# Arshardh/siddhi

Measured on AMD Instinct MI355X. Metric: events/sec (node) windowed group-by agg at 1/2/4/8 GPUs; % HBM roofline, higher is better.
Workload: dtype f64; 1 GPU; C2 timeBatch(1 sec) count/min/max/avg group by k, per-event sends; key_type=string (dictionary ids = dense slots), keys_per_gpu=100000, keys_total=100000, send_size=1, parallelism=key-sharded x1, flushes=69793, rows=6978983088

## Files before the change

siddhi_amd/csrc/sh_internal.h:

```cpp
#pragma once

#include <hip/hip_runtime.h>
#include <stdint.h>

#include "../../include/siddhi_hip.h"

namespace shd {

typedef unsigned long long u64;
typedef int64_t i64;
typedef unsigned int u32;

constexpr int kMaxFilterOps = 32;
constexpr int kBlock = 256;
constexpr int kItems = 8;
constexpr int kTile = kBlock * kItems;
constexpr u64 kEmptyKey = 0x8000000000000001ull;
constexpr u32 kNoPos = 0xFFFFFFFFu;
constexpr int kPackIdxBits = 22;
constexpr u32 kPackIdxMask = (1u << kPackIdxBits) - 1u;

struct FilterOpD {
    int op, type, col, pad;
    i64 ival;
// ... 156 lines not shown
                        WinParams wp, PushInfo* info, i64* blk_xm = nullptr, ColSet cols = ColSet{});
void launch_boundaries(hipStream_t s, const i64* ts, ColSet cols, FilterProg f, WinParams wp,
                       i64* blk_pass_pre, const i64* blk_tl_pre, PushInfo* info, Bound* bounds,
                       int max_bounds, int nblk, KeyPlan kp, KeyTable kt, u32* new_pos, const i64* blk_xm_pre = nullptr,
                       u32* ms_counts = nullptr, int P = 1, int ms_nblk = 0, int ms_col0 = 0, bool sorted = false,
                       i64* scan_tmp = nullptr);
int agg_unit_rows(int P, int NL, bool own);
void launch_aggregate(hipStream_t s, const Segment* segs, int nseg, int P, int logP, int NL, i64 n_pend,
                      const u32* pend_pos, const u64* pend_vals, i64 pend_cap, const u32* new_pos, ColSet cols,
                      AggPlan ap, u64* rows, int RW, u32* unit_rows, u32* first_bits,
                      const u32* rec_pos, const u32* rec_idx, const u64* rec_vals, i64 rec_cap, const i64* seg_off,
                      bool pack, EvSrc es, bool dense_rows = false,
                      bool persistent = true);
void launch_count_flags(hipStream_t s, const unsigned char* flags, i64 n, i64* blk_cnt, int nblk);
void launch_scan_sum(hipStream_t s, i64* a, int n);
void launch_bits_prefix(hipStream_t s, const u32* bits, i64 nw, i64* tile_sum, u64* word_pre, u32* total);
void launch_emit_rows(hipStream_t s, const u64* rows, int RW, const u32* unit_rows, i64 n_units, int unit_stride,
                      i64 row_cap, const u32* n_rows_dev, const u64* word_pre, int n_aggs, KeyTable kt,
                      KeyPlan kp, i64 n_pend, const i64* pend_ts, const i64* ts, i64 out_cap, i64* out_ts,
                      i64* out_keys, u64* out_vals, const u64* pend_gidx, const u64* new_gidx, i64* out_order,
                      i64 seq_base, i64* out_rep, u64* stage);
size_t emit_stage_bytes(int nk, int na, int order, i64 n_rows);
void launch_emit_gather(hipStream_t s, const u64* word_pre, i64 nw, const Segment* segs, int nseg, int P, int logP,
                        int unit_stride, const u64* rows, int RW, PosSrc ps, const u32* pend_pos, i64 n_pend,
                        const u32* n_rows_dev, int n_aggs, KeyTable kt, KeyPlan kp, i64* out_ts, i64* out_keys,
                        u64* out_vals, const u64* pend_gidx, const u64* new_gidx, i64* out_order, i64 seq_base,
                        i64* out_rep);
void launch_compact_pending(hipStream_t s, const i64* ts, ColSet cols, PosSrc new_pos, AggPlan ap, i64 e_lo,
                            i64 N, i64 pcb_lo, i64 base, const i64* blk_pass_pre, u32* pend_pos, i64* pend_ts,
                            u64* pend_vals, i64 pend_cap, const u64* new_gidx, u64* pend_gidx, i64 seq_base);
constexpr int kSmallT = 1024;
// ... 214 lines not shown
```

siddhi_amd/csrc/sh_kernels.hip:

```cpp
#include "sh_device.h"

namespace shd {

#ifdef SH_STAMPS
constexpr int kStampKernels = 4, kStampBlocks = 32768, kStampPts = 16;
__device__ unsigned long long g_stamps[kStampKernels * kStampBlocks * kStampPts];
#define SH_STAMP_AT(kern, idx, pt, WAIT)                                                                     \
    do {                                                                                                     \
        if (threadIdx.x == 0 && (idx) < kStampBlocks) {                                                      \
            asm volatile(WAIT ::: "memory");                                                                 \
            g_stamps[((size_t)(kern) * kStampBlocks + (idx)) * kStampPts + (pt)] = __builtin_amdgcn_s_memtime(); \
        }                                                                                                    \
    } while (0)
#define SH_STAMP(kern, pt) SH_STAMP_AT(kern, blockIdx.x, pt, "s_waitcnt vmcnt(0) lgkmcnt(0)")
#define SH_STAMP_UNIT(kern, unit, pt) SH_STAMP_AT(kern, unit, pt, "s_waitcnt vmcnt(0) lgkmcnt(0)")
#define SH_STAMP_UNIT_LDS(kern, unit, pt) SH_STAMP_AT(kern, unit, pt, "s_waitcnt lgkmcnt(0)")
#else
#define SH_STAMP(kern, pt) do {} while (0)
#define SH_STAMP_UNIT(kern, unit, pt) do {} while (0)
#define SH_STAMP_UNIT_LDS(kern, unit, pt) do {} while (0)
#endif

template <int FK>
__global__ __launch_bounds__(kBlock) void k_blockagg(const i64* __restrict__ ts, ColSet cols, FilterProg f,
// ... 899 lines not shown

void launch_scan_sum(hipStream_t s, i64* a, int n) {
    hipLaunchKernelGGL(k_scan_sum, dim3(1), dim3(1024), 0, s, a, n);
}

__global__ __launch_bounds__(kBlock) void k_bits_tile(const u32* __restrict__ bits, i64 nw, i64* tile_sum) {
    const i64 base = (i64)blockIdx.x * kTile + (i64)threadIdx.x * kItems;
    i64 c = 0;
#pragma unroll
    for (int i = 0; i < kItems; i++) if (base + i < nw) c += __popc(bits[base + i]);
    const i64 t = block_reduce(c, SumOp(), 0);
    if (threadIdx.x == 0) tile_sum[blockIdx.x] = t;
}

__global__ __launch_bounds__(kBlock) void k_bits_pre(const u32* __restrict__ bits, i64 nw, const i64* tile_pre,
                                                    u64* word_pre, u32* total) {
    const i64 base = (i64)blockIdx.x * kTile + (i64)threadIdx.x * kItems;
    u32 b[kItems];
    i64 c = 0;
#pragma unroll
    for (int i = 0; i < kItems; i++) { b[i] = base + i < nw ? bits[base + i] : 0; c += __popc(b[i]); }
    i64 r = block_excl_scan(c, SumOp(), 0, nullptr) + tile_pre[blockIdx.x];
#pragma unroll
    for (int i = 0; i < kItems; i++) {
        if (base + i < nw) word_pre[base + i] = ((u64)b[i] << 32) | (u32)r;
        r += __popc(b[i]);
        if (base + i == nw - 1) *total = (u32)r;
    }
}

void launch_bits_prefix(hipStream_t s, const u32* bits, i64 nw, i64* tile_sum, u64* word_pre, u32* total) {
    const int nb = (int)((nw + kTile - 1) / kTile);
    hipLaunchKernelGGL(k_bits_tile, dim3(nb), dim3(kBlock), 0, s, bits, nw, tile_sum);
    launch_scan_sum(s, tile_sum, nb);
    hipLaunchKernelGGL(k_bits_pre, dim3(nb), dim3(kBlock), 0, s, bits, nw, tile_sum, word_pre, total);
}

__host__ __device__ constexpr int stage_words(int nk, int na, int order) { return (2 + nk + order + na + 1) & ~1; }

constexpr int kStageMax = 2 + kKeyParts + 1 + SH_MAX_AGGS + 1;
__global__ __launch_bounds__(kBlock) void k_emit_rank(const u64* __restrict__ rows, int RW,
                                                     const u32* __restrict__ unit_rows, i64 n_units,
                                                     int unit_stride,
                                                     const u64* __restrict__ word_pre,
                                                     int n_aggs, KeyTable kt, KeyPlan kp, i64 n_pend,
                                                     const i64* __restrict__ pend_ts, const i64* __restrict__ ts,
                                                     const u64* __restrict__ pend_gidx,
                                                     const u64* __restrict__ new_gidx, int want_order, i64 seq_base,
                                                     u64* stage) {
    __shared__ ulonglong2 sw[kBlock][kStageMax / 2];
// ... 506 lines not shown
    if (p <= P) part_off[p] = counts[(i64)p * nblk];
}

void launch_part_off(hipStream_t s, const i64* counts, int nblk, int P, i64* part_off) {
    hipLaunchKernelGGL(k_part_off, dim3((P + 1 + 255) / 256), dim3(256), 0, s, counts, nblk, P, part_off);
}

constexpr int kColT = 16;
__global__ __launch_bounds__(kBlock) void k_col_reduce(const u32* __restrict__ c, int nblk, int P, i64* bsum,
                                                      u32* ticket) {
    const int b = blockIdx.y;
    const int p = blockIdx.x * kBlock + threadIdx.x;
    if (b == 0 && p == 0) *ticket = 0;
    if (p >= P) return;
    const int t0 = b * kColT, t1 = min(nblk, t0 + kColT);
    i64 acc = 0;
    for (int t = t0; t < t1; t++) acc += c[(i64)t * P + p];
    bsum[(i64)b * P + p] = acc;
}

__global__ __launch_bounds__(kBlock) void k_col_blocks(i64* bsum, int nb, int P, i64* total, i64* base, u32* ticket) {
    const int p = blockIdx.x;
    i64 run = 0;
    for (int b0 = 0; b0 < nb; b0 += kBlock) {
        const int b = b0 + threadIdx.x;
        const i64 x = b < nb ? bsum[(i64)b * P + p] : 0;
        i64 tot;
        const i64 pre = block_excl_scan(x, SumOp(), 0, &tot);
        if (b < nb) bsum[(i64)b * P + p] = run + pre;
        run += tot;
    }
    __shared__ bool last;
    if (threadIdx.x == 0) {
        total[p] = run;
        __threadfence();
        last = atomicAdd(ticket, 1u) == (u32)(P - 1);
    }
    __syncthreads();
    if (!last) return;
    __threadfence();
    i64 carry = 0;
    for (int q0 = 0; q0 < P; q0 += kBlock) {
        const int q = q0 + threadIdx.x;
        const i64 x = q < P ? __atomic_load_n(&total[q], __ATOMIC_RELAXED) : 0;
        i64 tot;
        const i64 pre = block_excl_scan(x, SumOp(), 0, &tot);
        if (q < P) base[q] = carry + pre;
        carry += tot;
    }
}

__global__ __launch_bounds__(kBlock) void k_col_walk(i64* __restrict__ bsum, int nb, int P, i64* __restrict__ total,
                                                    i64* __restrict__ base) {
    const int p = blockIdx.x * kBlock + threadIdx.x;
    if (p >= P) return;
    i64 run = 0;
    for (int b0 = 0; b0 < nb; b0 += 8) {
        i64 x[8];
#pragma unroll
        for (int k = 0; k < 8; k++) x[k] = b0 + k < nb ? bsum[(i64)(b0 + k) * P + p] : 0;
#pragma unroll
        for (int k = 0; k < 8; k++) {
            if (b0 + k < nb) bsum[(i64)(b0 + k) * P + p] = run;
            run += x[k];
        }
    }
    total[p] = run;
    base[p] = run;
}

__global__ __launch_bounds__(kBlock) void k_col_apply(u32* c, int nblk, int P, const i64* __restrict__ bpre,
                                                     const i64* __restrict__ base, const i64* __restrict__ total) {
    const int b = blockIdx.y;
    const int p = blockIdx.x * kBlock + threadIdx.x;
    if (p >= P) return;
    const int t0 = b * kColT, t1 = min(nblk, t0 + kColT);
    i64 run = base[p] + bpre[(i64)b * P + p];
    for (int t = t0; t < t1; t++) {
        const u32 x = c[(i64)t * P + p];
        c[(i64)t * P + p] = (u32)run;
        run += x;
    }
    if (t1 == nblk) c[(i64)nblk * P + p] = (u32)(base[p] + total[p]);
}

size_t ms_offsets_tmp_bytes(int nblk, int P) {
    const size_t nb = (size_t)(std::max(nblk, 1) + kColT - 1) / kColT;
    return (nb * P + 2 * (size_t)P + 16) * 8;
}

void launch_ms_offsets(hipStream_t s, u32* counts, int nblk, int P, i64* tmp) {
    const int nb = (std::max(nblk, 1) + kColT - 1) / kColT;
    i64* bsum = tmp;
    i64* total = tmp + (size_t)nb * P;
    i64* base = total + P;
    u32* ticket = (u32*)(base + P);
    const dim3 g((P + kBlock - 1) / kBlock, nb);
    hipLaunchKernelGGL(k_col_reduce, g, dim3(kBlock), 0, s, counts, nblk, P, bsum, ticket);
    if (P >= 2048 && nb <= 256) {
        hipLaunchKernelGGL(k_col_walk, dim3((P + kBlock - 1) / kBlock), dim3(kBlock), 0, s, bsum, nb, P, total, base);
        launch_scan_sum(s, base, P);
    } else {
        hipLaunchKernelGGL(k_col_blocks, dim3(P), dim3(kBlock), 0, s, bsum, nb, P, total, base, ticket);
    }
    if (nblk > 0) hipLaunchKernelGGL(k_col_apply, g, dim3(kBlock), 0, s, counts, nblk, P, bsum, base, total);
    else hipLaunchKernelGGL(k_col_apply, dim3((P + kBlock - 1) / kBlock, 1), dim3(kBlock), 0, s, counts, nblk, P, bsum,
                            base, total);
}

__global__ __launch_bounds__(kBlock) void k_seg_offsets(const Segment* __restrict__ segs, int nseg, i64 n_pend,
                                                       const u32* __restrict__ pend_pos,
                                                       PosSrc new_pos, int P,
                                                       const u32* __restrict__ counts, TileMap m, i64* seg_off) {
    extern __shared__ __attribute__((aligned(16))) u32 hist[];
    const int k = blockIdx.x;
    const i64 b = k < nseg ? segs[k].lo : segs[nseg - 1].hi;
    const int t = tile_of(m, b);
    for (int i = threadIdx.x; i < P; i += kBlock) hist[i] = 0;
// ... 636 lines not shown
```

siddhi_amd/csrc/sh_runtime.cpp:

```cpp
#include <hip/hip_runtime.h>

#include <algorithm>
#include <cstdio>
#include <cstdlib>
#include <cstring>
#include <string>
#include <vector>

#include "sh_agg.h"
#include "sh_internal.h"
#include "sh_runtime.h"

#include <chrono>

using namespace shd;

thread_local std::string g_last_error;

int sh_fail(int code, const std::string& msg) {
    g_last_error = msg;
    SH_TRACE("error %d: %s", code, msg.c_str());
    return code;
}

// ... 93 lines not shown
}

void DevBuf::release() {
    if (p) {
        (void)drain();
        (void)hipFree(p);
    }
    p = nullptr;
    cap = used = 0;
}

int PinnedBuf::reserve(size_t n) {
    if (n <= cap) return SH_OK;
    release();
    size_t ncap = std::max<size_t>(n, 4096);
    if (hipHostMalloc(&p, ncap, hipHostMallocDefault) != hipSuccess) {
        p = nullptr;
        return sh_fail(SH_ERR_OOM, "pinned host allocation failed");
    }
    cap = ncap;
    return SH_OK;
}

void PinnedBuf::release() {
    if (p) (void)hipHostFree(p);
    p = nullptr;
    cap = 0;
}

extern "C" int sh_init(int32_t device, sh_ctx** out) {
    if (!out) return sh_fail(SH_ERR_INVALID, "sh_init: out is NULL");
    int n = 0;
    hipError_t e = hipGetDeviceCount(&n);
    if (e != hipSuccess || n == 0) return sh_fail(SH_ERR_DEVICE, "no HIP device visible (this library has no CPU path)");
    if (device < 0 || device >= n) return sh_fail(SH_ERR_INVALID, "sh_init: bad device ordinal");
    HIPCHK(hipSetDevice(device));
    hipDeviceProp_t prop;
    HIPCHK(hipGetDeviceProperties(&prop, device));
    if (std::string(prop.gcnArchName).find("gfx950") == std::string::npos)
        return sh_fail(SH_ERR_DEVICE, std::string("built for gfx950, found ") + prop.gcnArchName);
    hipMemPool_t pool = nullptr;
// ... 287 lines not shown
```

siddhi_amd/csrc/sh_runtime.h:

```cpp
#pragma once

#include <hip/hip_runtime.h>
#include <rocprofiler-sdk-roctx/roctx.h>

#include <algorithm>
#include <cstdio>
#include <new>
#include <utility>
#include <string>
#include <unordered_map>
#include <vector>

#include "sh_internal.h"
#include "sh_having.h"

struct sh_ctx {
    int device = 0;
    int num_cus = 0;
    int max_lds = 0;
    hipStream_t stream = nullptr;
    hipStream_t copy_stream = nullptr;
    hipStream_t side_stream = nullptr;
};

// ... 49 lines not shown
            release();
            p = o.p; cap = o.cap; used = o.used;
            o.p = nullptr; o.cap = o.used = 0;
        }
        return *this;
    }
    ~DevBuf() { release(); }
    int reserve(size_t n, bool keep);
    void release();
    template <typename T> T* as() const { return (T*)p; }
};

struct PinnedBuf {
    void* p = nullptr;
    size_t cap = 0;
    PinnedBuf() = default;
    PinnedBuf(const PinnedBuf&) = delete;
    PinnedBuf& operator=(const PinnedBuf&) = delete;
    PinnedBuf(PinnedBuf&& o) noexcept : p(o.p), cap(o.cap) { o.p = nullptr; o.cap = 0; }
    PinnedBuf& operator=(PinnedBuf&& o) noexcept {
        if (this != &o) {
            release();
            p = o.p; cap = o.cap;
            o.p = nullptr; o.cap = 0;
        }
        return *this;
    }
    ~PinnedBuf() { release(); }
    int reserve(size_t n);
    void release();
    template <typename T> T* as() const { return (T*)p; }
};

struct KeyTableHost {
    DevBuf keys, ctrl;
    PinnedBuf h_ctrl;
    size_t size_ = 0;
    int64_t n_keys = 0;
    bool reserved_used = false;
// ... 158 lines not shown
    DevBuf pend_pos, pend_ts, pend_vals;
    DevBuf pend_tmp;
    DevBuf sp_pos, sp_ts, sp_vals, sp_gidx;
    int64_t sp_cap = 0;
    bool side_push = false;
    DevBuf blk_pass, blk_tl, blk_first, blk_xm, info, bounds, segs, seg_rows, rows, counters, out_ts, out_keys, out_vals,
        out_nulls, out_expired, out_rep, blk_cnt;
    DevBuf first_bits, word_pre;
    DevBuf emit_stage;
    const void* zeroed_nulls = nullptr;
    const void* zeroed_expired = nullptr;
    DevBuf ms_counts, ms_tmp, rec_pos, rec_idx, rec_vals, part_off;
    DevBuf new_pos, seg_off;
    PushInfo* h_info = nullptr;
    PinnedBuf h_up;
    PinnedBuf h_tail;
    PinnedBuf h_bounds;
    bool ms_ready = false;
    bool rec_packed = false;
    bool direct_pos = false;
    const sh_batch* zc_host = nullptr;
    std::vector<int64_t> sc_sl_host;
    bool band_keys = false;
    bool band_spec = false;
    PinnedBuf h_spec;
    uint32_t band_lk = 0, band_rows = 0, band_mul = 1, band_add = 0;
    shd::SmallRes* small_res = nullptr;
    shd::SmallRes* small_res_dev = nullptr;
    uint64_t small_token = 0;
    static constexpr int kZcRing = 8;
    char* zc_ring = nullptr;
    char* zc_ring_dev = nullptr;
    size_t zc_slot = 0;
    uint64_t zc_tok[kZcRing]{};
    int zc_next = 0;
    uint64_t async_tok = 0;
    int64_t async_keys = 0;
    TileMap ms_map{};
    int64_t rec_cap = 0;
    struct ClosedTail {
        bool active = false, host_done = false;
        int nseg = 0, units_per_seg = 1;
        int64_t closed_hi = 0;
        std::vector<int64_t> clocks, windows;
    } tail;
    StagedBatch staged;
    OutHost out;
    sh_out dev_out{};
    PinnedVec<int64_t> dev_flush_offsets{0}, dev_flush_clock;
    hipEvent_t ev_push0 = nullptr, ev_push1 = nullptr, ev_agg0 = nullptr, ev_agg1 = nullptr;
    hipEvent_t ev_srt0 = nullptr, ev_srt1 = nullptr;
    bool srt_timed = false;
    hipEvent_t ev_mid = nullptr;
    hipEvent_t ev_cnt = nullptr, ev_ms_off = nullptr, ev_seg = nullptr, ev_cmp = nullptr;
    sh_stats stats{};
    int64_t agg_bytes = 0;
    std::vector<int64_t> flush_window;
    bool internal_keys = false;
    size_t kt_min_size = 0;
    int32_t load_type[SH_MAX_COLS]{};
    uint32_t cols_used = 0;
    bool given = false;
    const int* given_wcol = nullptr;
    const shd::u64* given_gidx = nullptr;
    const int64_t* given_clk = nullptr;
    int64_t given_seq0 = 0, given_ss = 1;
    int64_t given_W_base = 0, given_W_end = 0;
    std::vector<sh_bound> gbounds;
    DevBuf pend_gidx, out_order;
// ... 124 lines not shown
```

siddhi_amd/csrc/sh_window.cpp:

```cpp
#include <hip/hip_runtime.h>

#include <algorithm>
#include <atomic>
#include <cstdlib>
#include <cstring>
#include <string>
#include <vector>

#include "sh_agg.h"
#include "sh_internal.h"
#include "sh_runtime.h"
#include "sh_wide.h"

using namespace shd;

#define HIPCHK(x)                                                                                          \
    do {                                                                                                   \
        hipError_t _e = (x);                                                                               \
        if (_e != hipSuccess) return sh_fail(SH_ERR_DEVICE, std::string(#x) + ": " + hipGetErrorString(_e)); \
    } while (0)
#define RCHK(x)            \
    do {                   \
        int _r = (x);      \
        if (_r) return _r; \
// ... 452 lines not shown
        HIPCHK(hipMemsetAsync(q->out_expired.p, 0, cap, s));
        q->zeroed_expired = nullptr;
        uint32_t* unit_rows = (uint32_t*)(q->counters.as<char>() + 64);
        HIPCHK(hipEventRecord(q->ev_agg0, s));
        launch_pass_rows(s, closed_hi, q->n_pend, b ? q->new_pos.as<u32>() : nullptr, q->pass_pos.as<u32>(),
                         q->x_tmp.as<int64_t>(), q->pend_ts.as<int64_t>(), q->pend_gidx.as<u64>(), ts, q->seq,
                         q->segs.as<Segment>(), nseg, q->out_ts.as<int64_t>(), q->out_rep.as<int64_t>(), unit_rows,
                         q->counters.as<u32>());
        HIPCHK(hipGetLastError());
        HIPCHK(hipEventRecord(q->ev_agg1, s));
        RCHK(q->h_tail.reserve(16 + (size_t)nseg * 4));
        HIPCHK(hipMemcpyAsync(q->h_tail.as<char>() + 16, unit_rows, nseg * 4, hipMemcpyDeviceToHost, s));
        auto& t = q->tail;
        t.active = true;
        t.host_done = false;
        t.nseg = nseg;
        t.units_per_seg = 1;
        t.closed_hi = closed_hi;
        t.clocks = clocks;
        t.windows = windows;
        if (host_out) {
            HIPCHK(hipStreamSynchronize(s));
            RCHK(closed_finish(q, true));
        }
        return SH_OK;
    }
    int64_t row_cap = 0;
    for (auto& sg : segs) row_cap += std::min<int64_t>(sg.hi - sg.lo, (int64_t)q->kt.size_ + 1);
    row_cap = std::max<int64_t>(row_cap, 1);
    const int na = q->ap.n, nk = q->kp.n, RW = row_words(na);
// ... 42 lines not shown
                     gather, q->tune.fold_grid);
    HIPCHK(hipGetLastError());
    HIPCHK(hipEventRecord(q->ev_agg1, s));
    const int64_t cap = row_cap;
    RCHK(q->out_ts.reserve(cap * 8, false));
    RCHK(q->out_keys.reserve(std::max(1, nk) * cap * 8, false));
    RCHK(q->out_vals.reserve(na * cap * 8, false));
    RCHK(q->out_nulls.reserve(na * cap, false));
    RCHK(q->out_expired.reserve(cap, false));
    RCHK(q->out_rep.reserve(cap * 8, false));
    if (q->given) RCHK(q->out_order.reserve(cap * 8, false));
    const int nbt = (int)((n_words + kTile - 1) / kTile);
    RCHK(q->blk_cnt.reserve((nbt + 16) * 8, false));
    RCHK(q->word_pre.reserve((size_t)n_words * 8, false));
    if (!gather) RCHK(q->emit_stage.reserve(emit_stage_bytes(nk, na, q->given ? 1 : 0, cap), false));
    launch_bits_prefix(s, q->first_bits.as<u32>(), n_words, q->blk_cnt.as<int64_t>(), q->word_pre.as<u64>(),
                       q->counters.as<u32>());
    if (gather)
        launch_emit_gather(s, q->word_pre.as<u64>(), n_words, dsegs, nseg, q->P, q->logP, unit_stride, q->rows.as<u64>(),
                           RW, pos_src(q, b), q->pend_pos.as<u32>(), q->n_pend, q->counters.as<u32>(), na, q->kt.dev(),
                           q->kp, q->out_ts.as<int64_t>(), q->out_keys.as<int64_t>(), q->out_vals.as<u64>(),
                           q->pend_gidx.as<u64>(), q->given && b ? q->given_gidx : nullptr,
                           q->given ? q->out_order.as<int64_t>() : nullptr, q->seq, q->out_rep.as<int64_t>());
    else
        launch_emit_rows(s, q->rows.as<u64>(), RW, unit_rows, n_units, unit_stride, cap, q->counters.as<u32>(),
                         q->word_pre.as<u64>(), na, q->kt.dev(), q->kp, q->n_pend,
                         q->pend_ts.as<int64_t>(), ts, cap,
                         q->out_ts.as<int64_t>(), q->out_keys.as<int64_t>(), q->out_vals.as<u64>(), q->pend_gidx.as<u64>(),
                         q->given && b ? q->given_gidx : nullptr, q->given ? q->out_order.as<int64_t>() : nullptr, q->seq,
                         q->out_rep.as<int64_t>(), q->emit_stage.as<u64>());
    if (q->out_nulls.p != q->zeroed_nulls) {
        HIPCHK(hipMemsetAsync(q->out_nulls.p, 0, q->out_nulls.cap, s));
        q->zeroed_nulls = q->out_nulls.p;
    }
    if (q->out_expired.p != q->zeroed_expired) {
        HIPCHK(hipMemsetAsync(q->out_expired.p, 0, q->out_expired.cap, s));
        q->zeroed_expired = q->out_expired.p;
    }
    HIPCHK(hipGetLastError());
    RCHK(q->h_tail.reserve(16 + (size_t)n_units * 4));
    HIPCHK(hipMemcpyAsync(q->h_tail.as<char>() + 16, unit_rows, n_units * 4, hipMemcpyDeviceToHost, s));
    auto& t = q->tail;
    t.active = true;
    t.host_done = false;
    t.nseg = nseg;
    t.units_per_seg = own ? q->P : 1;
    t.closed_hi = closed_hi;
    t.clocks = clocks;
    t.windows = windows;
    SH_TRACE("run_closed queued");
    if (host_out) {
        HIPCHK(hipStreamSynchronize(s));
        RCHK(closed_finish(q, true));
    }
    return SH_OK;
}

static int closed_finish(sh_query* q, bool host_out) {
    auto& t = q->tail;
    if (!t.active || t.host_done) return SH_OK;
    t.host_done = true;
    hipStream_t s = q->ctx->stream;
    const uint32_t* unit_rows = (const uint32_t*)(q->h_tail.as<char>() + 16);
    std::vector<int64_t> seg_rows(t.nseg, 0);
    for (int i = 0; i < t.nseg; i++)
        for (int u = 0; u < t.units_per_seg; u++) seg_rows[i] += unit_rows[(size_t)i * t.units_per_seg + u];
    const int na = q->ap.n, nk = q->kp.n;
    int64_t n_rows = 0;
    for (int i = 0; i < t.nseg; i++) n_rows += seg_rows[i];
    float agg_ms = 0;
    (void)hipEventElapsedTime(&agg_ms, q->ev_agg0, q->ev_agg1);
    q->stats.main_kernel_ms += agg_ms;
    q->agg_bytes += t.closed_hi * (int64_t)(4 + 8 * q->ap.n_vcols) + n_rows * (int64_t)(8 * row_words(na));
    if (host_out && n_rows > 0) {
        size_t base = q->out.ts.size();
        size_t nb = base + n_rows;
        q->out.ts.resize(nb);
        q->out.expired.resize(nb, 0);
        q->out.rep.resize(nb);
        HIPCHK(hipMemcpyAsync(q->out.ts.data() + base, q->out_ts.p, n_rows * 8, hipMemcpyDeviceToHost, s));
        HIPCHK(hipMemcpyAsync(q->out.rep.data() + base, q->out_rep.p, n_rows * 8, hipMemcpyDeviceToHost, s));
// ... 48 lines not shown
    std::vector<Segment> segs{Segment{0, q->n_pend}};
    std::vector<int64_t> clocks{clock}, windows{q->W_open};
    RCHK(run_closed(q, segs, clocks, windows, nullptr, host_out));
    HIPCHK(hipStreamSynchronize(q->ctx->stream));
    return closed_finish(q, host_out);
}

static void reset_call_output(sh_query* q) {
    q->dev_flush_offsets.assign(1, 0);
    q->dev_flush_clock.clear();
    q->flush_window.clear();
    q->dev_out = sh_out{};
    q->ms_ready = false;
    q->side_push = false;
    q->tail.active = false;
}

int flush_layout_to_device(sh_query* q, sh_out& o) {
    if (!q->device_flushes || q->rate.kind != SH_RATE_NONE || q->wide || q->hv.on || !o.flush_offsets) return SH_OK;
    const size_t nf = (size_t)o.n_flushes;
    hipStream_t s = q->ctx->stream;
    RCHK(q->fl_dev.reserve((2 * nf + 1) * 8, false));
    HIPCHK(hipMemcpyAsync(q->fl_dev.p, o.flush_offsets, (nf + 1) * 8, hipMemcpyHostToDevice, s));
    if (nf) HIPCHK(hipMemcpyAsync(q->fl_dev.as<int64_t>() + nf + 1, o.flush_clock, nf * 8, hipMemcpyHostToDevice, s));
    HIPCHK(hipStreamSynchronize(s));
    o.flush_offsets = q->fl_dev.as<int64_t>();
    o.flush_clock = q->fl_dev.as<int64_t>() + nf + 1;
    return SH_OK;
}

// ... 85 lines not shown
}

int query_resize_for_restore(sh_query* q, size_t table_size, int64_t n_pend, const KeyBand* band) {
    if (band) {
        q->kt.release();
        RCHK(q->kt.init_band(band->lk, band->rows, band->base, q->band_mul, q->band_add));
        if (table_size != q->kt.size_) return sh_fail(SH_ERR_INVALID, "snapshot does not match this query");
    } else if (q->kt.dense && !q->kt.lk) {
        if (table_size != q->kt.size_) return sh_fail(SH_ERR_INVALID, "snapshot does not match this query");
    } else if (table_size != q->kt.size_ || q->kt.lk) {
        q->kt.release();
        RCHK(q->kt.init_size(table_size));
    }
    RCHK(size_partitions(q));
    q->n_pend = 0;
    return grow_pending(q, n_pend, 0);
}

static int pending_to_front(sh_query* q, int64_t lo, int64_t n) {
    if (lo == 0 || n == 0) return SH_OK;
    hipStream_t s = q->ctx->stream;
    const bool direct = lo >= n;
    if (!direct) RCHK(q->pend_tmp.reserve((size_t)n * 8, false));
    auto move = [&](void* base, size_t elem) -> int {
        if (direct) {
            HIPCHK(hipMemcpyAsync(base, (char*)base + (size_t)lo * elem, (size_t)n * elem, hipMemcpyDeviceToDevice, s));
            return SH_OK;
        }
        void* t = q->pend_tmp.p;
        HIPCHK(hipMemcpyAsync(t, (char*)base + (size_t)lo * elem, (size_t)n * elem, hipMemcpyDeviceToDevice, s));
// ... 301 lines not shown
    q->stats.events = N;
    *done = true;
    return SH_OK;
}

static void given_closes(sh_query* q);

static int xr_trim(sh_query* q);
static int push_core(sh_query* q, const sh_batch* b, bool host_out_req, const sh_out** out) {
    SH_TMARK(0);
    const bool host_out = host_out_req && !q->xmode;
    q->x_closes.clear();
    q->x_stamps.clear();
    hipStream_t s = q->ctx->stream;
    q->out.reset();
    reset_call_output(q);
    q->stats = sh_stats{};
    q->agg_bytes = 0;
    q->order_host.clear();
    int64_t N = b->n;
    const bool cv0 = q->clock_valid;
    const int64_t clock0 = q->clock, seq0 = q->seq;
    bool swap_spare = false;
    if (N < 0) return sh_fail(SH_ERR_INVALID, "negative batch size");
    if (N > 0 && (!b->ts)) return sh_fail(SH_ERR_INVALID, "batch without timestamps");
    if (q->n_pend + N >= (int64_t)0xFFFFFFF0ll) return sh_fail(SH_ERR_INVALID, "push larger than 4G events");
    RCHK(small_verify(q, false));
    if (N > 0 && !q->internal_keys && q->kt.n_keys + q->async_keys > (int64_t)q->kt.size_ / 2) {
        RCHK(small_verify(q, true));
        if (q->kt.n_keys > (int64_t)q->kt.size_ / 2) RCHK(query_reserve_keys(q, 0));
// ... 34 lines not shown
        }
        const bool single_pass = !ext && !q->given && wp.pcol1 == 0 && wp.kind == SH_WIN_TIME_BATCH && wp.e0_valid;
        int max_bounds = (int)std::min<int64_t>(N + 1, 1 << 22);
        constexpr size_t kInfoPad = 2 * sizeof(Bound);
        static_assert(sizeof(PushInfo) <= kInfoPad, "the info block must fit in front of the boundaries");
        RCHK(q->bounds.reserve(kInfoPad + (size_t)max_bounds * sizeof(Bound), false));
        PushInfo* const d_info = q->bounds.as<PushInfo>();
        Bound* const d_bounds = (Bound*)(q->bounds.as<char>() + kInfoPad);
        auto prefix_passes = [&] {
            launch_blockagg(s, b->ts, cs, q->fp, N, b->send_size, q->blk_pass.as<int64_t>(), q->blk_tl.as<int64_t>(),
                            q->blk_first.as<int64_t>(), nblk, ext ? q->blk_xm.as<int64_t>() : nullptr,
                            ext ? q->d.ts_col : -1);
            launch_scan_blocks(s, q->blk_pass.as<int64_t>(), q->blk_tl.as<int64_t>(), q->blk_first.as<int64_t>(), nblk,
                               b->ts, wp, d_info, ext ? q->blk_xm.as<int64_t>() : nullptr, cs);
        };
        if (single_pass) {
            RCHK(q->blk_pass.reserve((size_t)(nblk + 1) * 8, false));
            launch_zero2(s, d_info, (int)sizeof(PushInfo), q->blk_pass.as<int64_t>() + nblk, 8);
            HIPCHK(hipGetLastError());
        } else {
            prefix_passes();
        }
        q->direct_pos = want_direct_pos(q);
        if (!q->direct_pos) RCHK(q->new_pos.reserve((size_t)N * 4, false));
        u32* slot_col = q->direct_pos ? nullptr : q->new_pos.as<u32>();
        const bool early_split = (q->P > 1 || q->partitioned) && N >= (1 << 18) && !q->d.stream_current;
        const TileMap ms_map = make_tile_map(q->n_pend, q->n_pend + N);
        if (early_split) RCHK(reserve_ms_counts(q, ms_map));
        q->side_push = early_split && q->tune.side_stream && !q->hv.on && q->ap.n != 0 && !q->given && q->xt_timeout == 0;
        launch_boundaries(s, b->ts, cs, q->fp, wp, q->blk_pass.as<int64_t>(), q->blk_tl.as<int64_t>(),
                          d_info, d_bounds, max_bounds, nblk, q->kp, q->kt.dev(),
                          slot_col, ext ? q->blk_xm.as<int64_t>() : nullptr,
                          early_split ? q->ms_counts.as<u32>() : nullptr, q->P, ms_map.nblk, ms_map.np_t,
                          single_pass, q->blk_tl.as<int64_t>());
        HIPCHK(hipGetLastError());
        constexpr int kFirstBounds = 256;
        const int nb0 = (int)std::min<int64_t>(max_bounds, std::max<int64_t>(kFirstBounds, q->last_nb + q->last_nb / 4 + 64));
        const size_t first_bytes = kInfoPad + (size_t)nb0 * sizeof(Bound);
        RCHK(q->h_bounds.reserve(first_bytes));
        const Bound* const h_bounds = (const Bound*)(q->h_bounds.as<char>() + kInfoPad);
        HIPCHK(hipMemcpyAsync(q->h_bounds.p, q->bounds.p, first_bytes, hipMemcpyDeviceToHost, s));
        const bool rsv_probe = q->d.stream_current && !q->kt.dense && !q->kt.reserved_used;
        if (q->band_spec || rsv_probe) {
            RCHK(q->h_spec.reserve(16));
            RCHK(q->kt.check_async(s, q->h_spec.as<uint32_t>()));
        }
        HIPCHK(hipEventRecord(q->ev_mid, s));
        SH_TMARK(1);
        if (q->side_push && ms_map.np_t > 0) {
            hipStream_t ss = q->ctx->side_stream;
            HIPCHK(hipStreamWaitEvent(ss, q->ev_push0, 0));
            launch_ms_count(ss, ms_map, ms_map.np_t, q->n_pend, q->pend_pos.as<u32>(), pos_src(q, b), q->P,
                            q->ms_counts.as<u32>());
            HIPCHK(hipEventRecord(q->ev_cnt, ss));
        }
        if (early_split) RCHK(run_multisplit(q, q->n_pend + N, b, true));
        SH_TRACE("push N=%lld n_pend=%lld: boundaries queued", (long long)N, (long long)q->n_pend);
// ... 134 lines not shown
            HIPCHK(hipStreamWaitEvent(s, q->ev_cmp, 0));
            swap_spare = true;
        } else {
            RCHK(grow_pending(q, new_pend, dst_base));
            launch_compact_pending(s, b->ts, cs, pos_src(q, b), q->ap, e_lo, N, pcb_lo, dst_base,
                                   q->blk_pass.as<int64_t>(), q->pend_pos.as<u32>(), q->pend_ts.as<int64_t>(),
                                   q->pend_vals.as<u64>(), q->pend_cap, q->given ? q->given_gidx : nullptr,
                                   q->pend_gidx.as<u64>(), q->seq);
            HIPCHK(hipGetLastError());
        }
        q->n_pend = new_pend;
    }
    q->seq += N;
    HIPCHK(hipEventRecord(q->ev_push1, s));
    RCHK(q->h_tail.reserve(16));
    RCHK(q->kt.check_async(s, q->h_tail.as<uint32_t>()));
    SH_TRACE("push final sync");
    SH_TMARK(4);
    HIPCHK(sh_wait_stream(s));
    SH_TMARK(5);
    SH_TRACE("push done");
    if (swap_spare) swap_pending(q);
    q->side_push = false;
    RCHK(q->kt.check_result(q->h_tail.as<uint32_t>()));
    RCHK(closed_finish(q, host_out));
    float ms = 0;
    (void)hipEventElapsedTime(&ms, q->ev_push0, q->ev_push1);
    q->stats.push_ms = ms;
    q->stats.events = N;
    q->stats.main_kernel_bytes = q->agg_bytes;
    if (q->xmode) return xout_finish(q, host_out_req, out);
    RCHK(finish_out(q, host_out, out));
    SH_TMARK(6);
    return SH_OK;
}

int check_batch_cols(const sh_query* q, const sh_batch* b) {
    if (b->n <= 0) return SH_OK;
    const int nc = q->wide ? q->wide_n_cols : q->d.n_cols;
    const uint64_t used = q->wide ? q->wide_cols_used : q->cols_used;
    for (int c = 0; c < nc; c++)
        if ((used >> c & 1) && !b->cols[c])
            return sh_fail(SH_ERR_INVALID, "batch column " + std::to_string(c) + " is NULL but the query reads it");
    return SH_OK;
}

extern "C" int sh_push(sh_query* q, const sh_batch* b, const sh_out** out) {
// ... 420 lines not shown
```

Baseline: 35.73 billion events/s.

## Fold tail readback and next-push zeroing into bits-prefix kernel, parallelize column scan

The bits-prefix kernel now computes per-segment row ranks and writes them, together with the key-table control words, straight into a device-mapped pinned host buffer. This replaces a separate device-to-host memcpy and a check_async copy. The same kernel pre-zeroes the next push's info and tail regions, so the following push can skip its zero launch when the buffers are unchanged. The per-column block scan is rewritten as a 1024-thread multi-column kernel, and the column reduce and apply loops are register-unrolled. These changes aim to cut small-launch and copy overhead on each flush, at the cost of extra state tracking and coherent-memory writes from the GPU.

```diff
diff --git a/siddhi_amd/csrc/sh_internal.h b/siddhi_amd/csrc/sh_internal.h
--- a/siddhi_amd/csrc/sh_internal.h
+++ b/siddhi_amd/csrc/sh_internal.h
@@ -194,7 +194,18 @@
                       bool persistent = true);
 void launch_count_flags(hipStream_t s, const unsigned char* flags, i64 n, i64* blk_cnt, int nblk);
 void launch_scan_sum(hipStream_t s, i64* a, int n);
-void launch_bits_prefix(hipStream_t s, const u32* bits, i64 nw, i64* tile_sum, u64* word_pre, u32* total);
+struct TailOut {
+    const Segment* segs;
+    int nseg;
+    u32* seg_rank;
+    const u32* ctrl;
+    u32* h_ctrl;
+    u32* zero_info;
+    int zero_words;
+    u32* zero_tail;
+};
+void launch_bits_prefix(hipStream_t s, const u32* bits, i64 nw, i64* tile_sum, u64* word_pre, u32* total,
+                        TailOut to = TailOut{});
 void launch_emit_rows(hipStream_t s, const u64* rows, int RW, const u32* unit_rows, i64 n_units, int unit_stride,
                       i64 row_cap, const u32* n_rows_dev, const u64* word_pre, int n_aggs, KeyTable kt,
                       KeyPlan kp, i64 n_pend, const i64* pend_ts, const i64* ts, i64 out_cap, i64* out_ts,
diff --git a/siddhi_amd/csrc/sh_kernels.hip b/siddhi_amd/csrc/sh_kernels.hip
--- a/siddhi_amd/csrc/sh_kernels.hip
+++ b/siddhi_amd/csrc/sh_kernels.hip
@@ -937,7 +937,7 @@
 }
 
 __global__ __launch_bounds__(kBlock) void k_bits_pre(const u32* __restrict__ bits, i64 nw, const i64* tile_pre,
-                                                    u64* word_pre, u32* total) {
+                                                    u64* word_pre, u32* total, TailOut to) {
     const i64 base = (i64)blockIdx.x * kTile + (i64)threadIdx.x * kItems;
     u32 b[kItems];
     i64 c = 0;
@@ -950,13 +950,37 @@
         r += __popc(b[i]);
         if (base + i == nw - 1) *total = (u32)r;
     }
-}
-
-void launch_bits_prefix(hipStream_t s, const u32* bits, i64 nw, i64* tile_sum, u64* word_pre, u32* total) {
+    if (!to.seg_rank) return;
+    __syncthreads();
+    const i64 e_lo = (i64)blockIdx.x * kTile * 32, e_hi = min(nw, (i64)(blockIdx.x + 1) * kTile) * 32;
+    const int n_ends = 2 * to.nseg;
+    int first = 0;
+    for (int hi = n_ends; first < hi;) {
+        const int mid = (first + hi) >> 1;
+        const i64 e = mid & 1 ? to.segs[mid >> 1].hi : to.segs[mid >> 1].lo;
+        if (e < e_lo) first = mid + 1;
+        else hi = mid;
+    }
+    for (int i = first + threadIdx.x; i < n_ends; i += kBlock) {
+        const i64 e = i & 1 ? to.segs[i >> 1].hi : to.segs[i >> 1].lo;
+        if (e >= e_hi) break;
+        const i64 w = e >> 5;
+        const u64 wp = __atomic_load_n(&word_pre[w], __ATOMIC_RELAXED);
+        to.seg_rank[i] = (u32)wp + (u32)__popc((u32)(wp >> 32) & ((1u << (e & 31)) - 1u));
+    }
+    if (blockIdx.x != 0) return;
+    if (threadIdx.x < 4) to.h_ctrl[threadIdx.x] = to.ctrl[threadIdx.x];
+    if (to.zero_info) {
+        for (int i = threadIdx.x; i < to.zero_words; i += kBlock) to.zero_info[i] = 0;
+        if (threadIdx.x < 2) to.zero_tail[threadIdx.x] = 0;
+    }
+}
+
+void launch_bits_prefix(hipStream_t s, const u32* bits, i64 nw, i64* tile_sum, u64* word_pre, u32* total, TailOut to) {
     const int nb = (int)((nw + kTile - 1) / kTile);
     hipLaunchKernelGGL(k_bits_tile, dim3(nb), dim3(kBlock), 0, s, bits, nw, tile_sum);
     launch_scan_sum(s, tile_sum, nb);
-    hipLaunchKernelGGL(k_bits_pre, dim3(nb), dim3(kBlock), 0, s, bits, nw, tile_sum, word_pre, total);
+    hipLaunchKernelGGL(k_bits_pre, dim3(nb), dim3(kBlock), 0, s, bits, nw, tile_sum, word_pre, total, to);
 }
 
 __host__ __device__ constexpr int stage_words(int nk, int na, int order) { return (2 + nk + order + na + 1) & ~1; }
@@ -1493,39 +1517,94 @@
     if (b == 0 && p == 0) *ticket = 0;
     if (p >= P) return;
     const int t0 = b * kColT, t1 = min(nblk, t0 + kColT);
+    u32 x[kColT];
+#pragma unroll
+    for (int k = 0; k < kColT; k++) x[k] = t0 + k < t1 ? c[(i64)(t0 + k) * P + p] : 0u;
     i64 acc = 0;
-    for (int t = t0; t < t1; t++) acc += c[(i64)t * P + p];
+#pragma unroll
+    for (int k = 0; k < kColT; k++) acc += x[k];
     bsum[(i64)b * P + p] = acc;
 }
 
-__global__ __launch_bounds__(kBlock) void k_col_blocks(i64* bsum, int nb, int P, i64* total, i64* base, u32* ticket) {
-    const int p = blockIdx.x;
+constexpr int kLineT = 1024, kLineP = 16, kLineU = 8, kLineKeep = 24;
+__global__ __launch_bounds__(kLineT) void k_col_lines(i64* bsum, int nb, int P, i64* total, i64* base, u32* ticket) {
+    __shared__ i64 gsum[kLineT];
+    __shared__ bool last;
+    const int t = threadIdx.x;
+    const int lw = min(P, kLineP), G = kLineT / lw;
+    const int l = t & (lw - 1), g = t / lw;
+    const int p = blockIdx.x * lw + l;
+    const int rpt = (nb + G - 1) / G;
+    const int r0 = min(nb, g * rpt), r1 = min(nb, r0 + rpt);
+    i64* const col = bsum + p;
+    const bool keep = rpt <= kLineKeep;
+    u32 x[kLineKeep];
+    i64 acc = 0;
+    if (keep) {
+#pragma unroll
+        for (int k = 0; k < kLineKeep; k++) x[k] = r0 + k < r1 ? (u32)col[(i64)(r0 + k) * P] : 0u;
+#pragma unroll
+        for (int k = 0; k < kLineKeep; k++) acc += x[k];
+    } else {
+        for (int r = r0; r < r1; r += kLineU) {
+            i64 y[kLineU];
+#pragma unroll
+            for (int k = 0; k < kLineU; k++) y[k] = r + k < r1 ? col[(i64)(r + k) * P] : 0;
+#pragma unroll
+            for (int k = 0; k < kLineU; k++) acc += y[k];
+        }
+    }
+    gsum[t] = acc;
+    __syncthreads();
     i64 run = 0;
-    for (int b0 = 0; b0 < nb; b0 += kBlock) {
-        const int b = b0 + threadIdx.x;
-        const i64 x = b < nb ? bsum[(i64)b * P + p] : 0;
-        i64 tot;
-        const i64 pre = block_excl_scan(x, SumOp(), 0, &tot);
-        if (b < nb) bsum[(i64)b * P + p] = run + pre;
-        run += tot;
-    }
-    __shared__ bool last;
-    if (threadIdx.x == 0) {
+    if (G <= 64) {
+        for (int k = 0; k < g; k++) run += gsum[k * lw + l];
+    } else {
+        for (int d = lw; d < kLineT; d <<= 1) {
+            const i64 v = t >= d ? gsum[t - d] : 0;
+            __syncthreads();
+            gsum[t] += v;
+            __syncthreads();
+        }
+        run = gsum[t] - acc;
+    }
+    if (keep) {
+#pragma unroll
+        for (int k = 0; k < kLineKeep; k++) {
+            if (r0 + k < r1) col[(i64)(r0 + k) * P] = run;
+            run += x[k];
+        }
+    } else {
+        for (int r = r0; r < r1; r += kLineU) {
+            i64 y[kLineU];
+#pragma unroll
+            for (int k = 0; k < kLineU; k++) y[k] = r + k < r1 ? col[(i64)(r + k) * P] : 0;
+#pragma unroll
+            for (int k = 0; k < kLineU; k++) {
+                if (r + k < r1) col[(i64)(r + k) * P] = run;
+                run += y[k];
+            }
+        }
+    }
+    if (g == G - 1) {
         total[p] = run;
         __threadfence();
-        last = atomicAdd(ticket, 1u) == (u32)(P - 1);
+    }
+    __syncthreads();
+    if (t == 0) {
+        last = atomicAdd(ticket, 1u) == gridDim.x - 1;
+        if (last) __threadfence();
     }
     __syncthreads();
     if (!last) return;
-    __threadfence();
-    i64 carry = 0;
-    for (int q0 = 0; q0 < P; q0 += kBlock) {
-        const int q = q0 + threadIdx.x;
-        const i64 x = q < P ? __atomic_load_n(&total[q], __ATOMIC_RELAXED) : 0;
-        i64 tot;
-        const i64 pre = block_excl_scan(x, SumOp(), 0, &tot);
-        if (q < P) base[q] = carry + pre;
-        carry += tot;
+    const int per = (P + kLineT - 1) / kLineT;
+    const int q0 = min(P, t * per), q1 = min(P, q0 + per);
+    i64 mine = 0;
+    for (int q = q0; q < q1; q++) mine += __atomic_load_n(&total[q], __ATOMIC_RELAXED);
+    i64 pre = block_excl_scan_any(mine, nullptr);
+    for (int q = q0; q < q1; q++) {
+        base[q] = pre;
+        pre += __atomic_load_n(&total[q], __ATOMIC_RELAXED);
     }
 }
 
@@ -1555,10 +1634,13 @@
     if (p >= P) return;
     const int t0 = b * kColT, t1 = min(nblk, t0 + kColT);
     i64 run = base[p] + bpre[(i64)b * P + p];
-    for (int t = t0; t < t1; t++) {
-        const u32 x = c[(i64)t * P + p];
-        c[(i64)t * P + p] = (u32)run;
-        run += x;
+    u32 x[kColT];
+#pragma unroll
+    for (int k = 0; k < kColT; k++) x[k] = t0 + k < t1 ? c[(i64)(t0 + k) * P + p] : 0u;
+#pragma unroll
+    for (int k = 0; k < kColT; k++) {
+        if (t0 + k < t1) c[(i64)(t0 + k) * P + p] = (u32)run;
+        run += x[k];
     }
     if (t1 == nblk) c[(i64)nblk * P + p] = (u32)(base[p] + total[p]);
 }
@@ -1580,7 +1662,7 @@
         hipLaunchKernelGGL(k_col_walk, dim3((P + kBlock - 1) / kBlock), dim3(kBlock), 0, s, bsum, nb, P, total, base);
         launch_scan_sum(s, base, P);
     } else {
-        hipLaunchKernelGGL(k_col_blocks, dim3(P), dim3(kBlock), 0, s, bsum, nb, P, total, base, ticket);
+        hipLaunchKernelGGL(k_col_lines, dim3(P / std::min(P, kLineP)), dim3(kLineT), 0, s, bsum, nb, P, total, base, ticket);
     }
     if (nblk > 0) hipLaunchKernelGGL(k_col_apply, g, dim3(kBlock), 0, s, counts, nblk, P, bsum, base, total);
     else hipLaunchKernelGGL(k_col_apply, dim3((P + kBlock - 1) / kBlock, 1), dim3(kBlock), 0, s, counts, nblk, P, bsum,
diff --git a/siddhi_amd/csrc/sh_runtime.cpp b/siddhi_amd/csrc/sh_runtime.cpp
--- a/siddhi_amd/csrc/sh_runtime.cpp
+++ b/siddhi_amd/csrc/sh_runtime.cpp
@@ -131,8 +131,10 @@
     if (n <= cap) return SH_OK;
     release();
     size_t ncap = std::max<size_t>(n, 4096);
-    if (hipHostMalloc(&p, ncap, hipHostMallocDefault) != hipSuccess) {
-        p = nullptr;
+    if (hipHostMalloc(&p, ncap, mapped ? hipHostMallocMapped | hipHostMallocCoherent : hipHostMallocDefault) != hipSuccess ||
+        (mapped && hipHostGetDevicePointer(&dev, p, 0) != hipSuccess)) {
+        if (p) (void)hipHostFree(p);
+        p = dev = nullptr;
         return sh_fail(SH_ERR_OOM, "pinned host allocation failed");
     }
     cap = ncap;
@@ -141,7 +143,7 @@
 
 void PinnedBuf::release() {
     if (p) (void)hipHostFree(p);
-    p = nullptr;
+    p = dev = nullptr;
     cap = 0;
 }
 
diff --git a/siddhi_amd/csrc/sh_runtime.h b/siddhi_amd/csrc/sh_runtime.h
--- a/siddhi_amd/csrc/sh_runtime.h
+++ b/siddhi_amd/csrc/sh_runtime.h
@@ -87,15 +87,21 @@
 struct PinnedBuf {
     void* p = nullptr;
     size_t cap = 0;
+    bool mapped = false;
+    void* dev = nullptr;
     PinnedBuf() = default;
+    explicit PinnedBuf(bool device_mapped) : mapped(device_mapped) {}
     PinnedBuf(const PinnedBuf&) = delete;
     PinnedBuf& operator=(const PinnedBuf&) = delete;
-    PinnedBuf(PinnedBuf&& o) noexcept : p(o.p), cap(o.cap) { o.p = nullptr; o.cap = 0; }
+    PinnedBuf(PinnedBuf&& o) noexcept : p(o.p), cap(o.cap), mapped(o.mapped), dev(o.dev) {
+        o.p = o.dev = nullptr;
+        o.cap = 0;
+    }
     PinnedBuf& operator=(PinnedBuf&& o) noexcept {
         if (this != &o) {
             release();
-            p = o.p; cap = o.cap;
-            o.p = nullptr; o.cap = 0;
+            p = o.p; cap = o.cap; mapped = o.mapped; dev = o.dev;
+            o.p = o.dev = nullptr; o.cap = 0;
         }
         return *this;
     }
@@ -284,7 +290,7 @@
     DevBuf new_pos, seg_off;
     PushInfo* h_info = nullptr;
     PinnedBuf h_up;
-    PinnedBuf h_tail;
+    PinnedBuf h_tail{true};
     PinnedBuf h_bounds;
     bool ms_ready = false;
     bool rec_packed = false;
@@ -310,6 +316,7 @@
     int64_t rec_cap = 0;
     struct ClosedTail {
         bool active = false, host_done = false;
+        bool seg_ranks = false;
         int nseg = 0, units_per_seg = 1;
         int64_t closed_hi = 0;
         std::vector<int64_t> clocks, windows;
@@ -323,6 +330,15 @@
     bool srt_timed = false;
     hipEvent_t ev_mid = nullptr;
     hipEvent_t ev_cnt = nullptr, ev_ms_off = nullptr, ev_seg = nullptr, ev_cmp = nullptr;
+    struct HeadRegions {
+        void* info = nullptr;
+        void* tail = nullptr;
+        size_t info_cap = 0, tail_cap = 0;
+        bool same(const HeadRegions& o) const {
+            return info && info == o.info && tail == o.tail && info_cap == o.info_cap && tail_cap == o.tail_cap;
+        }
+    } head_clean, head_want;
+    bool head_queued = false;
     sh_stats stats{};
     int64_t agg_bytes = 0;
     std::vector<int64_t> flush_window;
diff --git a/siddhi_amd/csrc/sh_window.cpp b/siddhi_amd/csrc/sh_window.cpp
--- a/siddhi_amd/csrc/sh_window.cpp
+++ b/siddhi_amd/csrc/sh_window.cpp
@@ -490,6 +490,7 @@
         auto& t = q->tail;
         t.active = true;
         t.host_done = false;
+        t.seg_ranks = false;
         t.nseg = nseg;
         t.units_per_seg = 1;
         t.closed_hi = closed_hi;
@@ -562,8 +563,21 @@
     RCHK(q->blk_cnt.reserve((nbt + 16) * 8, false));
     RCHK(q->word_pre.reserve((size_t)n_words * 8, false));
     if (!gather) RCHK(q->emit_stage.reserve(emit_stage_bytes(nk, na, q->given ? 1 : 0, cap), false));
+    const bool tail_direct = side && gather;
+    RCHK(q->h_tail.reserve(16 + (size_t)std::max<int64_t>(n_units, 2 * (int64_t)nseg) * 4));
+    TailOut to{};
+    if (tail_direct) {
+        char* const d_tail = (char*)q->h_tail.dev;
+        to = TailOut{dsegs, nseg, (u32*)(d_tail + 16), (const u32*)q->kt.ctrl.p, (u32*)d_tail, nullptr, 0, nullptr};
+        if (q->head_want.info) {
+            to.zero_info = (u32*)q->head_want.info;
+            to.zero_words = (int)(sizeof(PushInfo) / 4);
+            to.zero_tail = (u32*)q->head_want.tail;
+            q->head_queued = true;
+        }
+    }
     launch_bits_prefix(s, q->first_bits.as<u32>(), n_words, q->blk_cnt.as<int64_t>(), q->word_pre.as<u64>(),
-                       q->counters.as<u32>());
+                       q->counters.as<u32>(), to);
     if (gather)
         launch_emit_gather(s, q->word_pre.as<u64>(), n_words, dsegs, nseg, q->P, q->logP, unit_stride, q->rows.as<u64>(),
                            RW, pos_src(q, b), q->pend_pos.as<u32>(), q->n_pend, q->counters.as<u32>(), na, q->kt.dev(),
@@ -586,11 +600,11 @@
         q->zeroed_expired = q->out_expired.p;
     }
     HIPCHK(hipGetLastError());
-    RCHK(q->h_tail.reserve(16 + (size_t)n_units * 4));
-    HIPCHK(hipMemcpyAsync(q->h_tail.as<char>() + 16, unit_rows, n_units * 4, hipMemcpyDeviceToHost, s));
+    if (!tail_direct) HIPCHK(hipMemcpyAsync(q->h_tail.as<char>() + 16, unit_rows, n_units * 4, hipMemcpyDeviceToHost, s));
     auto& t = q->tail;
     t.active = true;
     t.host_done = false;
+    t.seg_ranks = tail_direct;
     t.nseg = nseg;
     t.units_per_seg = own ? q->P : 1;
     t.closed_hi = closed_hi;
@@ -611,8 +625,13 @@
     hipStream_t s = q->ctx->stream;
     const uint32_t* unit_rows = (const uint32_t*)(q->h_tail.as<char>() + 16);
     std::vector<int64_t> seg_rows(t.nseg, 0);
-    for (int i = 0; i < t.nseg; i++)
+    for (int i = 0; i < t.nseg; i++) {
+        if (t.seg_ranks) {
+            seg_rows[i] = unit_rows[2 * i + 1] - unit_rows[2 * i];
+            continue;
+        }
         for (int u = 0; u < t.units_per_seg; u++) seg_rows[i] += unit_rows[(size_t)i * t.units_per_seg + u];
+    }
     const int na = q->ap.n, nk = q->kp.n;
     int64_t n_rows = 0;
     for (int i = 0; i < t.nseg; i++) n_rows += seg_rows[i];
@@ -691,6 +710,10 @@
     q->ms_ready = false;
     q->side_push = false;
     q->tail.active = false;
+    q->tail.seg_ranks = false;
+    q->head_clean = {};
+    q->head_want = {};
+    q->head_queued = false;
 }
 
 int flush_layout_to_device(sh_query* q, sh_out& o) {
@@ -806,6 +829,7 @@
     }
     RCHK(size_partitions(q));
     q->n_pend = 0;
+    q->head_clean = {};
     return grow_pending(q, n_pend, 0);
 }
 
@@ -1137,6 +1161,7 @@
     q->x_stamps.clear();
     hipStream_t s = q->ctx->stream;
     q->out.reset();
+    const sh_query::HeadRegions clean = q->head_clean;
     reset_call_output(q);
     q->stats = sh_stats{};
     q->agg_bytes = 0;
@@ -1201,10 +1226,14 @@
             launch_scan_blocks(s, q->blk_pass.as<int64_t>(), q->blk_tl.as<int64_t>(), q->blk_first.as<int64_t>(), nblk,
                                b->ts, wp, d_info, ext ? q->blk_xm.as<int64_t>() : nullptr, cs);
         };
+        sh_query::HeadRegions head;
         if (single_pass) {
             RCHK(q->blk_pass.reserve((size_t)(nblk + 1) * 8, false));
-            launch_zero2(s, d_info, (int)sizeof(PushInfo), q->blk_pass.as<int64_t>() + nblk, 8);
-            HIPCHK(hipGetLastError());
+            head = sh_query::HeadRegions{d_info, q->blk_pass.as<int64_t>() + nblk, q->bounds.cap, q->blk_pass.cap};
+            if (!head.same(clean)) {
+                launch_zero2(s, d_info, (int)sizeof(PushInfo), q->blk_pass.as<int64_t>() + nblk, 8);
+                HIPCHK(hipGetLastError());
+            }
         } else {
             prefix_passes();
         }
@@ -1215,6 +1244,7 @@
         const TileMap ms_map = make_tile_map(q->n_pend, q->n_pend + N);
         if (early_split) RCHK(reserve_ms_counts(q, ms_map));
         q->side_push = early_split && q->tune.side_stream && !q->hv.on && q->ap.n != 0 && !q->given && q->xt_timeout == 0;
+        if (q->side_push) q->head_want = head;
         launch_boundaries(s, b->ts, cs, q->fp, wp, q->blk_pass.as<int64_t>(), q->blk_tl.as<int64_t>(),
                           d_info, d_bounds, max_bounds, nblk, q->kp, q->kt.dev(),
                           slot_col, ext ? q->blk_xm.as<int64_t>() : nullptr,
@@ -1226,8 +1256,8 @@
         const size_t first_bytes = kInfoPad + (size_t)nb0 * sizeof(Bound);
         RCHK(q->h_bounds.reserve(first_bytes));
         const Bound* const h_bounds = (const Bound*)(q->h_bounds.as<char>() + kInfoPad);
+        const bool rsv_probe = q->d.stream_current && !q->kt.dense && !q->kt.reserved_used;
         HIPCHK(hipMemcpyAsync(q->h_bounds.p, q->bounds.p, first_bytes, hipMemcpyDeviceToHost, s));
-        const bool rsv_probe = q->d.stream_current && !q->kt.dense && !q->kt.reserved_used;
         if (q->band_spec || rsv_probe) {
             RCHK(q->h_spec.reserve(16));
             RCHK(q->kt.check_async(s, q->h_spec.as<uint32_t>()));
@@ -1392,7 +1422,7 @@
     q->seq += N;
     HIPCHK(hipEventRecord(q->ev_push1, s));
     RCHK(q->h_tail.reserve(16));
-    RCHK(q->kt.check_async(s, q->h_tail.as<uint32_t>()));
+    if (!(q->tail.active && q->tail.seg_ranks)) RCHK(q->kt.check_async(s, q->h_tail.as<uint32_t>()));
     SH_TRACE("push final sync");
     SH_TMARK(4);
     HIPCHK(sh_wait_stream(s));
@@ -1409,6 +1439,7 @@
     q->stats.main_kernel_bytes = q->agg_bytes;
     if (q->xmode) return xout_finish(q, host_out_req, out);
     RCHK(finish_out(q, host_out, out));
+    if (q->head_queued) q->head_clean = q->head_want;
     SH_TMARK(6);
     return SH_OK;
 }
```

Measured after the change: 37.57 billion events/s, median of 6. +5.1%, better.
